# NVlabs/bayes-sim-ig

Measured on AMD Instinct MI355X. Metric: summary_vectors_per_sec_in_fit, higher is better.
Workload: dtype f32; 1 GPU; cfg5: ShadowHand MDRFF-4096 K=4 D=32, summary_start (I=2310), 100000 pairs/GPU, reference chunk protocol: <=1000-pair chunks, summarizer + 100 Adam updates x minibatch 100 + 6 held-out evals per chunk; pairs_per_gpu=100000, parallelism=dp1, gradient_exchange=none, hip_graph=True

## Files before the change

bayes_sim_ig_amd/csrc/fit_deferred_eval.hip:

```cpp
#include "persist.h"

#include <algorithm>
#include <cstdlib>

#include "persist_linear_device.h"

namespace bsig {

struct DArgs {
  int e0, n_ev_chunk;
  float* slabs; int64_t slab_stride;
  float* rows; int row_floats;
  float* sx; float* sl;
};

__device__ __forceinline__ UEval d_eval_of(const UArgs& p, const DArgs& d, int gidx) {
  const int c = p.chunks ? gidx / d.n_ev_chunk : 0;
  return u_eval_of(p, c, gidx - c * d.n_ev_chunk);
}
__device__ __forceinline__ bool d_gave_up(const UArgs& p) {
  return (__hip_atomic_load(p.state + ST_FLAGS, __ATOMIC_RELAXED, __HIP_MEMORY_SCOPE_AGENT) & kFlagTimeout) != 0;
}
__device__ __forceinline__ float d_slot_sum(const float* vals, int n, int lane) {
  float v[4];
#pragma unroll
  for (int u = 0; u < 4; ++u) v[u] = lane + 64 * u < n ? vals[lane + 64 * u] : 0.f;
  return granule_slot_sum(v);
}

template <int NT>
__global__ __launch_bounds__(kUT) void deferred_eval_products_kernel(UArgs p, DArgs d) {
  extern __shared__ __attribute__((aligned(16))) float smem[];
#ifndef BSIG_HOST_SAN_BUILD
  if (d_gave_up(p)) return;
  constexpr int NBW = 16 * NT;
  float* Wl = smem;
  float* biasl = Wl + NBW * p.WP;
  const int tid = threadIdx.x;
  const int slot = blockIdx.x, gidx = d.e0 + blockIdx.y;
  const int ks = slot / p.n_blocks, nb = slot - ks * p.n_blocks;
  const float* src = p.snap + ((int64_t)gidx * p.G + slot) * u_snap_slot_floats(NT, p.WP);
  const int quads = NBW * p.WP / 4 + (ks == 0 ? NBW / 4 : 0);
  for (int i = tid; i < quads; i += kUT)
    *reinterpret_cast<f32x4*>(Wl + 4 * i) = *reinterpret_cast<const f32x4*>(src + 4 * i);
  __syncthreads();
  u_eval_products<NT>(p, Wl, biasl, ks, nb * NBW, ks * p.KS, d_eval_of(p, d, gidx), d.slabs + blockIdx.y * d.slab_stride);
#endif
}

__global__ __launch_bounds__(kUT) void deferred_eval_rows_kernel(UArgs p, DArgs d) {
  extern __shared__ __attribute__((aligned(16))) float smem[];
#ifndef BSIG_HOST_SAN_BUILD
  if (d_gave_up(p)) return;
  float* XS = smem;
  float* red = XS + d.row_floats;
  const int tid = threadIdx.x;
  const int eo = blockIdx.x, y = blockIdx.y;
  for (int i = tid; i < d.row_floats; i += kUT) XS[i] = 0.f;
  __syncthreads();
  const float sx = u_eval_rows(p, d.slabs + y * d.slab_stride, XS, red, eo, d_eval_of(p, d, d.e0 + y), tid);
  if (tid == 0) d.sx[y * p.NE + eo] = sx;
  float* out = d.rows + ((int64_t)y * p.NE + eo) * d.row_floats;
  for (int i = tid; i < d.row_floats; i += kUT) out[i] = XS[i];
#endif
}

__global__ __launch_bounds__(kUT) void deferred_eval_nll_kernel(UArgs p, DArgs d) {
  extern __shared__ __attribute__((aligned(16))) float smem[];
#ifndef BSIG_HOST_SAN_BUILD
  if (d_gave_up(p)) return;
  float* XS = smem;
  float* red = XS + d.row_floats;
  const int tid = threadIdx.x, lane = tid & 63;
  const int eo = blockIdx.x, y = blockIdx.y;
  const float* in = d.rows + ((int64_t)y * p.NE + eo) * d.row_floats;
  for (int i = tid; i < d.row_floats; i += kUT) XS[i] = in[i];
  __syncthreads();
  bool bad;
  const float sl = u_eval_nll(p, XS, red, eo, d_eval_of(p, d, d.e0 + y), u_head_args(p), tid,
                              [&] { return d_slot_sum(d.sx + y * p.NE, p.NE, lane); }, bad);
  if (tid == 0) d.sl[y * p.NE + eo] = sl;
  if (bad) atomicOr(p.state + ST_FLAGS, kFlagNonfinite);
#endif
}

__global__ __launch_bounds__(64) void deferred_eval_log_kernel(UArgs p, DArgs d, int n) {
#ifndef BSIG_HOST_SAN_BUILD
  if (d_gave_up(p)) return;
  const int lane = threadIdx.x;
  for (int y = 0; y < n; ++y) {
    const float sum = d_slot_sum(d.sl + y * p.NE, p.NE, lane);
    if (lane == 0) u_eval_log(p, d_eval_of(p, d, d.e0 + y), sum, p.state + ST_FLAGS);
  }
#endif
}

namespace {
struct DLayout { size_t snap_off, snap_bytes, slab_off, rows_off, sx_off, sl_off, total; int group; size_t slab_stride; int row_floats; };

DLayout d_layout(const UGeom& g, int n_evals) {
  DLayout L{};
  L.snap_off = 256;
  L.snap_bytes = round_up<size_t>(deferred_eval_snapshot_bytes(g, n_evals), 256);
  L.slab_stride = (size_t)std::max(g.eval_passes, 1) * g.slab_floats;
  L.group = (int)std::max<size_t>(1, std::min<size_t>({(size_t)n_evals, (size_t)64,
                                                      kDeferredGroupBytes / std::max<size_t>(L.slab_stride * sizeof(float), 1)}));
  L.row_floats = (int)round_up(g.RE * g.per_wave, 4);
  L.slab_off = L.snap_off + L.snap_bytes;
  L.rows_off = L.slab_off + round_up<size_t>((size_t)L.group * L.slab_stride * sizeof(float), 256);
  L.sx_off = L.rows_off + round_up<size_t>((size_t)L.group * g.NE * L.row_floats * sizeof(float), 256);
  L.sl_off = L.sx_off + round_up<size_t>((size_t)L.group * g.NE * sizeof(float), 256);
  L.total = L.sl_off + round_up<size_t>((size_t)L.group * g.NE * sizeof(float), 256);
  return L;
}
}

size_t deferred_eval_snapshot_bytes(const UGeom& g, int n_evals) {
  return (size_t)n_evals * g.G * (size_t)u_snap_slot_floats(g.NT, g.WP) * sizeof(float);
}

bool deferred_eval_reserve(const UGeom& g, int n_evals, DeferredEval* d) {
  if (n_evals < 1 || g.eval_passes < 1) return false;
  size_t cap = kDeferredSnapCapBytes;
  if (const char* e = getenv("BSIG_DEFERRED_EVAL_CAP_MB")) cap = (size_t)std::max(atoll(e), 0ll) << 20;
  if (deferred_eval_snapshot_bytes(g, n_evals) > cap) return false;
  if (d->mem && d->n_evals >= n_evals) return true;
  const DLayout L = d_layout(g, n_evals);
  if (d->mem) {
    if (hipDeviceSynchronize() != hipSuccess || hipFree(d->mem) != hipSuccess) return false;
    *d = DeferredEval{};
  }
  void* mem = nullptr;
  if (hipMalloc(&mem, L.total) != hipSuccess) {
    (void)hipGetLastError();
    return false;
  }
  d->mem = mem; d->bytes = L.total; d->n_evals = n_evals;
  return true;
}

void deferred_eval_free(DeferredEval* d) {
  if (d->mem) (void)hipFree(d->mem);
  *d = DeferredEval{};
}

int deferred_eval_run(const PersistShape& s, const UGeom& g, const PersistBuffers& b, int n, hipStream_t st) {
  BSIG_REQUIRE(b.deferred && b.do_eval && n >= 1, "deferred evaluations: not a launch with snapshots");
  UArgs p;
  BSIG_TRY(persist_fill_args(s, g, b, n, &p));
  const int n_ev_chunk = (int)count_logging_points(n);
  const int n_evals = n_ev_chunk * (b.chunks ? b.n_chunks : 1);
  const DLayout L = d_layout(g, n_evals);
  char* base = reinterpret_cast<char*>(b.deferred);
  DArgs d{};
  d.n_ev_chunk = n_ev_chunk;
  d.slabs = reinterpret_cast<float*>(base + L.slab_off); d.slab_stride = (int64_t)L.slab_stride;
  d.rows = reinterpret_cast<float*>(base + L.rows_off); d.row_floats = L.row_floats;
  d.sx = reinterpret_cast<float*>(base + L.sx_off); d.sl = reinterpret_cast<float*>(base + L.sl_off);
  const size_t lds_tile = (size_t)u_snap_slot_floats(g.NT, g.WP) * sizeof(float);
  const size_t lds_rows = ((size_t)L.row_floats + 64) * sizeof(float);
  BSIG_REQUIRE(lds_tile <= kLdsUnraised && lds_rows <= kLdsUnraised, "deferred evaluations: tile or rows beyond 64 KB of LDS");
  for (int e0 = 0; e0 < n_evals; e0 += L.group) {
    const int ne = std::min(L.group, n_evals - e0);
    d.e0 = e0;
    if (g.NT == 1)
      hipLaunchKernelGGL((deferred_eval_products_kernel<1>), dim3(g.G, ne), dim3(kUT), lds_tile, st, p, d);
    else
      hipLaunchKernelGGL((deferred_eval_products_kernel<2>), dim3(g.G, ne), dim3(kUT), lds_tile, st, p, d);
    BSIG_CHECK_LAUNCH("deferred_eval_products");
    hipLaunchKernelGGL(deferred_eval_rows_kernel, dim3(g.NE, ne), dim3(kUT), lds_rows, st, p, d);
    BSIG_CHECK_LAUNCH("deferred_eval_rows");
    hipLaunchKernelGGL(deferred_eval_nll_kernel, dim3(g.NE, ne), dim3(kUT), lds_rows, st, p, d);
    BSIG_CHECK_LAUNCH("deferred_eval_nll");
    hipLaunchKernelGGL(deferred_eval_log_kernel, dim3(1), dim3(64), 0, st, p, d, ne);
    BSIG_CHECK_LAUNCH("deferred_eval_log");
  }
  return BSIG_OK;
}

}
```

bayes_sim_ig_amd/csrc/persist.h:

```cpp
#pragma once
#include "common.h"

namespace bsig {

struct PersistEngine {
  int kind = 0;
  bool streams = false;
  bool eval_single = false;
  bool eval_dp = false;
  bool block_launch = false;
  size_t workspace_bytes = 0;
};

inline bool block_launch_resolved(int kind, bool eval_single, bool forced_single) {
  return kind == 1 && eval_single && !forced_single;
}

struct PersistShape {
  int batch, feat_dim, out_dim, n_comp;
  int max_test = 0;
};

struct UGeom {
  int NT, Bp, MT, FP, KS, ksteps, KB, WP, Nh, NhP, n_blocks, k_slices, G, T, n_owner, R;
  int per_wave, xs_floats;
  int eval_passes, NE, RE;
  size_t lds, slab_floats, dout_floats, eval_floats;
};

struct PersistHyper {
  double lr, beta1, beta2; float adam_eps, eps_noise, min_weight, ll_limit;
  int64_t norm_batch;
};

struct PersistCommon {
  const float* y; int64_t ldy;
  const int32_t* ids;
  float* params; float* exp_avg; float* exp_avg_sq;
  int32_t* state;
  float* train_loss;
  void* workspace; size_t workspace_bytes;
  float* grads = nullptr; int adam_pending = 0;
  unsigned* xr_ready = nullptr; const unsigned* xr_done = nullptr; unsigned xr_base = 0;
  int do_eval = 0; int eval_every = 1; int n_total = 0; int n_test = 0;
  const float* y_test = nullptr; int64_t ldy_test = 0;
  float* test_loss = nullptr;
  PersistHyper hy;
};

struct PersistBuffers : PersistCommon {
  const float* feats; int64_t ld_feats;
  const int32_t* feat_ids;
  int64_t w_off, b_off;
  int64_t eval_row0 = 0;
  const bsig_fit_chunk* chunks = nullptr; int n_chunks = 1;
  void* deferred = nullptr;
};

struct DeferredEval { void* mem = nullptr; size_t bytes = 0; int n_evals = 0; };
constexpr size_t kDeferredSnapCapBytes = (size_t)2 << 30;
constexpr size_t kDeferredGroupBytes = (size_t)96 << 20;
size_t deferred_eval_snapshot_bytes(const UGeom& g, int n_evals);
bool deferred_eval_reserve(const UGeom& g, int n_evals, DeferredEval* d);
void deferred_eval_free(DeferredEval* d);
int deferred_eval_run(const PersistShape& s, const UGeom& g, const PersistBuffers& b, int n, hipStream_t st);

bool persist_resolve(const PersistShape& s, UGeom* g, PersistEngine* e);
struct ZeroRegion { void* ptr; size_t bytes; };
int persist_reset_regions(const UGeom& g, void* workspace, size_t workspace_bytes, ZeroRegion* regions);
int persist_run(const PersistShape& s, const UGeom& g, const PersistBuffers& b, int n, hipStream_t st);

int persist_geometry(const PersistShape& s, int32_t* out);

template <int N>
inline int allow_dynamic_lds(LdsRaised (&raised)[N], const void* const (&kernels)[N], int bytes) {
  for (int i = 0; i < N; ++i) BSIG_TRY(raise_lds_limit(kernels[i], bytes, &raised[i]));
  return BSIG_OK;
}

void persist_set_profile_buffer(void* buf);
int debug_spin(int blocks, size_t lds_bytes, int ms, hipStream_t st);
void* persist_profile_buffer();

}
```

bayes_sim_ig_amd/csrc/persist_linear_device.h:

```cpp
#pragma once
#include "persist.h"
#include "head_device.h"
#include "persist_device.h"

namespace bsig {

constexpr int kUT = 512;
constexpr int kUSteps = 18;
constexpr int kUGroup = 6;
constexpr int kUMT = 7;
constexpr int kUProf = 8;
constexpr int kUFP = 116;

struct UArgs {
  int B, Bp, MT;
  int Fdim, KS, ksteps, KB, WP;
  int Nh, NhP, D, K;
  int n_blocks, k_slices, G, T, n_owner, R;
  int n_updates, xs_floats;
  int fast_rows;
  const float* feats; int64_t ld_feats; const int32_t* feat_ids;
  const float* y; int64_t ldy; const int32_t* ids;
  float* params; float* m1; float* m2; int64_t w_off, b_off;
  int32_t* state; float* train_loss;
  double lr, beta1, beta2;
  float adam_eps, eps_noise, min_w, ll_limit, inv_norm;
  float* slabs; float* d_out; float* e_out; unsigned* flag_fwd; unsigned long long* gran;
  unsigned long long* gran_rep;
  float* grads; int adam_pending; int quad_ok;
  unsigned* xr_ready; const unsigned* xr_done; unsigned* xr_count; unsigned xr_base;
  int do_eval, eval_every, n_total, n_test, eval_passes, NE, RE;
  int64_t eval_row0;
  const float* y_test; int64_t ldy_test;
  float* test_loss;
  float* eval_slabs;
  unsigned* flag_eval;
  unsigned long long* gran_eval;
  long long* prof;
  int prof_t0;
  const bsig_fit_chunk* chunks; int n_chunks;
  float* snap;
  const int32_t* state_in;
};
int persist_fill_args(const PersistShape& s, const UGeom& g, const PersistBuffers& b, int n, UArgs* out);
__host__ __device__ inline int64_t u_snap_slot_floats(int NT, int WP) { return (int64_t)16 * NT * (WP + 1); }

struct UCk {
  int step0, n_updates, n_total, eval_every, do_eval;
  unsigned ubase, evbase;
  uint64_t seed, rng_ctr0;
};
__device__ __forceinline__ int u_uniform(int v) { return __builtin_amdgcn_readfirstlane(v); }
__device__ __forceinline__ int64_t u_uniform(int64_t v) {
  return (int64_t)(((uint64_t)(uint32_t)u_uniform((int)((uint64_t)v >> 32)) << 32) | (uint32_t)u_uniform((int)(uint64_t)v));
}
__device__ __forceinline__ void u_chunk_load(const UArgs& p, int c, UCk& k) {
  if (p.chunks == nullptr) {
    k.step0 = p.state[ST_STEP]; k.n_updates = p.n_updates; k.n_total = p.n_total; k.eval_every = p.eval_every;
    k.do_eval = p.do_eval; k.ubase = 0u; k.evbase = 0u;
    k.seed = st_rng(p.state)[0];
    k.rng_ctr0 = st_rng(p.state)[1];
    return;
  }
  const bsig_fit_chunk& e = p.chunks[c];
  k.step0 = 0; k.n_updates = u_uniform(e.n_updates); k.n_total = k.n_updates; k.eval_every = u_uniform(e.eval_every);
  k.do_eval = 1; k.ubase = (unsigned)u_uniform(e.upd_base); k.evbase = (unsigned)u_uniform(e.eval_base);
  k.seed = (uint64_t)u_uniform((int64_t)e.seed); k.rng_ctr0 = (uint64_t)u_uniform((int64_t)e.rng_ctr0);
}

struct UEval {
  int n_test, passes; int64_t row0;
  const float* y_test; int64_t ldy_test;
  float* out;
  unsigned gidx;
  uint64_t seed, stream;
};
__device__ __forceinline__ UEval u_eval_of(const UArgs& p, int c, int e) {
  UEval v;
  int every, n_total, step0;
  uint64_t ctr0;
  if (p.chunks == nullptr) {
    v.n_test = p.n_test; v.row0 = p.eval_row0; v.y_test = p.y_test; v.ldy_test = p.ldy_test; v.out = nullptr;
    v.gidx = (unsigned)e; every = p.eval_every; n_total = p.n_total; step0 = p.state_in[ST_STEP];
    v.seed = st_rng(p.state_in)[0];
    ctr0 = st_rng(p.state_in)[1];
  } else {
    const bsig_fit_chunk& k = p.chunks[c];
    v.n_test = u_uniform(k.n_test); v.row0 = u_uniform(k.row0) + u_uniform(k.n_train);
    v.y_test = p.y + v.row0 * p.ldy; v.ldy_test = p.ldy; v.out = p.test_loss + u_uniform(k.test_slot) + e;
    v.gidx = (unsigned)u_uniform(k.eval_base) + (unsigned)e; every = u_uniform(k.eval_every);
    n_total = u_uniform(k.n_updates); step0 = 0;
    v.seed = (uint64_t)u_uniform((int64_t)k.seed); ctr0 = (uint64_t)u_uniform((int64_t)k.rng_ctr0);
  }
  v.passes = (v.n_test + p.B - 1) / p.B;
  const int at = eval_at_step(e, every, n_total);
  const int ev0 = p.do_eval || p.chunks ? evals_before(step0, every) : 0;
  v.stream = launch_stream(ctr0, at - step0, e, ev0);
  return v;
}

__device__ __forceinline__ f32x4 umfma(float a, float b, f32x4 c) {
  return __builtin_amdgcn_mfma_f32_16x16x4f32(a, b, c, 0, 0, 0);
}

template <typename RowOff, typename F>
__device__ __forceinline__ void u_rows_sum(const float* slabs, RowOff&& rowoff, int k_slices, int zs, int nrows,
                                           int n_cols, float* out, int out_pitch, int tid, F&& fn) {
  const __amdgpu_buffer_rsrc_t sr = xwg_buffer(slabs);
  for (int idx = tid; idx < nrows * n_cols; idx += kUT) {
    const int r = idx / n_cols, col = idx - r * n_cols;
    const int voff = (rowoff(r) + col) * 4;
    float v = 0.f;
    for (int z = 0; z < k_slices; z += 16) {
      float q[16];
#pragma unroll
      for (int u = 0; u < 16; ++u)
        q[u] = __uint_as_float(__builtin_amdgcn_raw_buffer_load_b32(sr, voff, min(z + u, k_slices - 1) * zs * 4, kXwgPolicy));
#pragma unroll
      for (int u = 0; u < 16; ++u)
        if (z + u < k_slices) v += q[u];
    }
    out[r * out_pitch + col] = v;
    fn(col, v);
  }
}


template <int NT>
__device__ __forceinline__ void u_eval_products(const UArgs& p, const float* Wl, const float* biasl, int ks, int n0,
                                                int k0, const UEval& ev, float* ebase) {
  int tid = threadIdx.x;
  asm volatile("" : "+v"(tid));
  const int lane = tid & 63, w = tid >> 6, c16 = lane & 15, g4 = lane >> 4;
  const int B = p.B, NhP = p.NhP;
  for (int pass = 0; pass < ev.passes; ++pass) {
    const int rows = min(B, ev.n_test - pass * B);
    if (rows <= 0) break;
    if (w < p.MT) {
      f32x4 acc[NT];
#pragma unroll
      for (int nt = 0; nt < NT; ++nt) {
        const f32x4 zero = {0.f, 0.f, 0.f, 0.f};
        acc[nt] = ks == 0 ? *reinterpret_cast<const f32x4*>(biasl + 16 * nt + 4 * g4) : zero;
      }
      const int64_t r = ev.row0 + pass * B + min(16 * w + c16, rows - 1);
      const float* src = p.feats + r * p.ld_feats;
      const float* ap = Wl + c16 * p.WP + 4 * g4;
#pragma unroll 1
      for (int s0 = 0; s0 < p.ksteps; s0 += kUGroup) {
        f32x4 breg[kUGroup];
#pragma unroll
        for (int q = 0; q < kUGroup; ++q) {
          const int col = k0 + 16 * (s0 + q) + 4 * g4;
          const f32x4 v = *reinterpret_cast<const f32x4*>(src + min((int64_t)col, p.ld_feats - 4));
          const f32x4 zero = {0.f, 0.f, 0.f, 0.f};
          breg[q] = col < p.Fdim ? v : zero;
        }
#pragma unroll
        for (int q = 0; q < kUGroup; ++q) {
#pragma unroll
          for (int nt = 0; nt < NT; ++nt) {
            const f32x4 a4 = *reinterpret_cast<const f32x4*>(ap + nt * 16 * p.WP + 16 * (s0 + q));
            acc[nt] = umfma(a4[0], breg[q][0], acc[nt]);
            acc[nt] = umfma(a4[1], breg[q][1], acc[nt]);
            acc[nt] = umfma(a4[2], breg[q][2], acc[nt]);
            acc[nt] = umfma(a4[3], breg[q][3], acc[nt]);
          }
        }
      }
      if (16 * w + c16 < rows) {
        const __amdgpu_buffer_rsrc_t sr = xwg_buffer(ebase + (((int64_t)pass * p.k_slices + ks) * B) * NhP + n0);
#pragma unroll
        for (int nt = 0; nt < NT; ++nt)
          xwg_store4(sr, (16 * w + c16) * NhP + 16 * nt + 4 * g4, acc[nt][0], acc[nt][1], acc[nt][2], acc[nt][3]);
      }
    }
  }
}

__device__ __forceinline__ float u_eval_rows(const UArgs& p, const float* ebase, float* XS, float* red, int eo,
                                             const UEval& ev, int tid) {
  const int lane = tid & 63, w = tid >> 6;
  const int B = p.B, Nh = p.Nh, NhP = p.NhP, K = p.K, DK = p.D * p.K;
  const int per_wave = Nh + p.D + 3 * K;
  const int nr = eo < ev.n_test ? min(p.RE, (ev.n_test - eo + p.NE - 1) / p.NE) : 0;
  float eacc = 0.f;
  u_rows_sum(ebase,
             [&](int r) {
               const int erow = eo + p.NE * r, pass = erow / B, rb = erow - pass * B;
               return (pass * p.k_slices * B + rb) * NhP;
             },
             p.k_slices, B * NhP, nr, Nh, XS, per_wave, tid,
             [&](int col, float v) { if (col >= K + DK && col < K + 2 * DK) eacc += expf(v); });
  eacc = wave_sum_dpp(eacc);
  if (lane == 0) red[w] = eacc;
  __syncthreads();
  float sx = 0.f;
  if (tid == 0)
    for (int q = 0; q < kUT / 64; ++q) sx += red[q];
  return sx;
}

template <typename SumExp>
__device__ __forceinline__ float u_eval_nll(const UArgs& p, float* XS, float* red, int eo, const UEval& ev,
                                            const HeadArgs& a, int tid, SumExp&& sum_exp, bool& bad) {
  const int lane = tid & 63, w = tid >> 6;
  const int Nh = p.Nh, D = p.D, K = p.K, DK = D * K;
  const int per_wave = Nh + D + 3 * K;
  const int nr = eo < ev.n_test ? min(p.RE, (ev.n_test - eo + p.NE - 1) / p.NE) : 0;
  const int erow = eo + p.NE * w;
  const bool act = w < nr;
  float* tile = XS + w * per_wave;
  float* yv = tile + Nh;
  float* rk = yv + D;
  float* lpk = rk + K;
  float* dlg = lpk + K;
  if (act)
    for (int j = lane; j < D; j += 64) yv[j] = ev.y_test[(int64_t)erow * ev.ldy_test + j];
  RowOut ro;
  ro.lse = 0.f; ro.uds = 0.f; ro.bad = false;
#pragma unroll
  for (int q = 0; q < kElemsPerLane; ++q) ro.esg0[q] = 0.f;
  if (w < p.RE) {
    HeadArgs ae = a;
    ae.d_out = nullptr;
    ae.batch = ev.n_test;
    ae.seed = ev.seed;
    ae.stream_id = ev.stream;
    diag_row(ae, erow, act, lane, tile, yv, rk, lpk, dlg,
             [&] {
               return p.eps_noise != 0.f ? p.eps_noise * (sum_exp() / ((float)ev.n_test * (float)DK)) : 0.f;
             },
             ro);
  }
  if (lane == 0) red[16 + w] = act ? ro.lse : 0.f;
  __syncthreads();
  float sl = 0.f;
  if (tid == 0)
    for (int q = 0; q < kUT / 64; ++q) sl += red[16 + q];
  bad = ro.bad;
  return sl;
}

__device__ __forceinline__ void u_eval_log(const UArgs& p, const UEval& ev, float sum, int32_t* flagp) {
  const float l = -sum / (float)ev.n_test;
  if (ev.out) *ev.out = l;
  else p.test_loss[p.state[ST_EVAL]] = l;
  p.state[ST_EVAL] = p.state[ST_EVAL] + 1;
  if (!isfinite(l)) atomicOr(flagp, kFlagNonfinite);
}

__device__ __forceinline__ HeadArgs u_head_args(const UArgs& p) {
  HeadArgs a{};
  a.D = p.D; a.K = p.K; a.Nh = p.Nh; a.batch = p.B; a.from_tuple = 0;
  a.min_w = p.min_w; a.ll_limit = p.ll_limit; a.inv_norm = p.inv_norm;
  a.eps_noise = p.eps_noise; a.d_out = p.d_out;
  return a;
}

template <int NT>
__device__ __forceinline__ void u_tile_eval(const UArgs& p, const float* Wl, const float* biasl, int slot,
                                            int ks, int n0, int k0, const UEval& ev) {
  u_eval_products<NT>(p, Wl, biasl, ks, n0, k0, ev,
                      p.eval_slabs + (int64_t)(ev.gidx % 3u) * p.eval_passes * p.k_slices * p.B * p.NhP);
  __builtin_amdgcn_s_waitcnt(0);
  __syncthreads();
  if (threadIdx.x == 0) flag_raise(p.flag_eval, slot, ev.gidx + 1u);
}

__device__ __forceinline__ void u_owner_eval(const UArgs& p, float* XS, float* red, int eo, const UEval& ev,
                                             const HeadArgs& a) {
  int tid = threadIdx.x;
  asm volatile("" : "+v"(tid));
  const int lane = tid & 63, w = tid >> 6;
  int32_t* flagp = p.state + ST_FLAGS;
  const unsigned etag = ev.gidx + 1u;
  if (w == 0) flags_wait(p.flag_eval, p.G, etag, lane, flagp);
  __syncthreads();
  const float* ebase = p.eval_slabs + (int64_t)(ev.gidx % 3u) * p.eval_passes * p.k_slices * p.B * p.NhP;
  const float sx = u_eval_rows(p, ebase, XS, red, eo, ev, tid);
  if (tid == 0) granule_publish(p.gran_eval, eo, etag, sx);
  bool bad;
  const float sl = u_eval_nll(p, XS, red, eo, ev, a, tid,
                              [&] { return granule_gather(p.gran_eval, p.NE, etag, lane, flagp); }, bad);
  if (tid == 0) granule_publish(p.gran_eval + kGranArr, eo, etag, sl);
  if (eo == 0 && w == 0) {
    const float sum = granule_gather(p.gran_eval + kGranArr, p.NE, etag, lane, flagp);
    if (lane == 0) u_eval_log(p, ev, sum, flagp);
  }
  if (bad) atomicOr(flagp, kFlagNonfinite);
  __syncthreads();
}

}
```

Measured before the change: 584,400 pairs/s.

## Restructure deferred eval products to reduce k-slices in-block with double-buffered tiles

The deferred-evaluation products kernel now launches one block per (eval, row group, n-block). Each block loops over all k-slices, streaming the weight tiles through double-buffered LDS with register prefetch and software-pipelined feature loads. It accumulates the k-slice partial sums in registers and writes one reduced sums buffer, instead of per-k-slice slabs that the rows kernel previously summed. The smaller intermediate lets group sizes grow (up to 4096 evals), which cuts launches, and the log kernel is parallelized across evals when chunked. The cost is less grid parallelism over k-slices and more register pressure.

New measurement: 588,200 pairs/s (median of 2 runs). About the same (+0.6%).

```diff
diff --git a/bayes_sim_ig_amd/csrc/fit_deferred_eval.hip b/bayes_sim_ig_amd/csrc/fit_deferred_eval.hip
--- a/bayes_sim_ig_amd/csrc/fit_deferred_eval.hip
+++ b/bayes_sim_ig_amd/csrc/fit_deferred_eval.hip
@@ -7,9 +7,14 @@
 
 namespace bsig {
 
+constexpr int kDRounds = 2;
+constexpr int kDRows = 16 * kDRounds * (kUT / 64);
+constexpr int kDQuads = 4;
+
 struct DArgs {
-  int e0, n_ev_chunk;
-  float* slabs; int64_t slab_stride;
+  int e0, n, n_ev_chunk;
+  int n_rg, lds_bufs;
+  float* sums; int64_t sum_stride;
   float* rows; int row_floats;
   float* sx; float* sl;
 };
@@ -34,17 +39,97 @@
 #ifndef BSIG_HOST_SAN_BUILD
   if (d_gave_up(p)) return;
   constexpr int NBW = 16 * NT;
-  float* Wl = smem;
-  float* biasl = Wl + NBW * p.WP;
-  const int tid = threadIdx.x;
-  const int slot = blockIdx.x, gidx = d.e0 + blockIdx.y;
-  const int ks = slot / p.n_blocks, nb = slot - ks * p.n_blocks;
-  const float* src = p.snap + ((int64_t)gidx * p.G + slot) * u_snap_slot_floats(NT, p.WP);
-  const int quads = NBW * p.WP / 4 + (ks == 0 ? NBW / 4 : 0);
-  for (int i = tid; i < quads; i += kUT)
-    *reinterpret_cast<f32x4*>(Wl + 4 * i) = *reinterpret_cast<const f32x4*>(src + 4 * i);
+  const int tid = threadIdx.x, lane = tid & 63, w = u_uniform(tid >> 6), c16 = lane & 15, g4 = lane >> 4;
+  const int item = blockIdx.x;
+  const int y = item / (d.n_rg * p.n_blocks), rg = (item - y * d.n_rg * p.n_blocks) / p.n_blocks;
+  const int nb = item - (y * d.n_rg + rg) * p.n_blocks;
+  const int gidx = d.e0 + y;
+  const UEval ev = d_eval_of(p, d, gidx);
+  const int rows = min(kDRows, ev.n_test - rg * kDRows);
+  if (rows <= 0) return;
+  const int n_mt = (rows + 15) / 16;
+  const int mt[kDRounds] = {w, kUT / 64 + w};
+  const bool has[kDRounds] = {mt[0] < n_mt, mt[1] < n_mt};
+  const int64_t slot_floats = u_snap_slot_floats(NT, p.WP);
+  const float* tiles = p.snap + ((int64_t)gidx * p.G + nb) * slot_floats;
+  const int64_t tile_step = (int64_t)p.n_blocks * slot_floats;
+  const float* biasl = smem + NBW * p.WP;
+  f32x4 pre[kDQuads];
+  auto tile_request = [&](int ks) {
+    const int quads = NBW * p.WP / 4 + (ks == 0 ? NBW / 4 : 0);
+    const float* src = tiles + ks * tile_step;
+#pragma unroll
+    for (int u = 0; u < kDQuads; ++u) {
+      const int i = tid + u * kUT;
+      if (i < quads) pre[u] = *reinterpret_cast<const f32x4*>(src + 4 * i);
+    }
+  };
+  auto tile_to_lds = [&](int ks) {
+    const int quads = NBW * p.WP / 4 + (ks == 0 ? NBW / 4 : 0);
+    float* dst = smem + (ks & (d.lds_bufs - 1)) * slot_floats;
+#pragma unroll
+    for (int u = 0; u < kDQuads; ++u) {
+      const int i = tid + u * kUT;
+      if (i < quads) *reinterpret_cast<f32x4*>(dst + 4 * i) = pre[u];
+    }
+  };
+  tile_request(0);
+  const int64_t row0 = ev.row0 + rg * kDRows;
+  const float* frow[kDRounds];
+#pragma unroll
+  for (int r = 0; r < kDRounds; ++r) frow[r] = u_slice_row(p, row0, rows, 16 * mt[r] + c16);
+  f32x4 cur[kUGroup];
+  u_slice_operands(p, frow[0], 0, 0, g4, cur);
+  tile_to_lds(0);
   __syncthreads();
-  u_eval_products<NT>(p, Wl, biasl, ks, nb * NBW, ks * p.KS, d_eval_of(p, d, gidx), d.slabs + blockIdx.y * d.slab_stride);
+  f32x4 sum[kDRounds][NT];
+#pragma unroll
+  for (int r = 0; r < kDRounds; ++r)
+#pragma unroll
+    for (int nt = 0; nt < NT; ++nt) sum[r][nt] = f32x4{0.f, 0.f, 0.f, 0.f};
+#pragma unroll 1
+  for (int ks = 0; ks < p.k_slices; ++ks) {
+    const bool more = ks + 1 < p.k_slices;
+    const int k0 = ks * p.KS;
+    if (more) tile_request(ks + 1);
+    const float* ap = smem + (ks & (d.lds_bufs - 1)) * slot_floats + c16 * p.WP + 4 * g4;
+#pragma unroll
+    for (int r = 0; r < kDRounds; ++r) {
+      if (!has[r]) continue;
+      f32x4 acc[NT];
+      u_slice_start<NT>(biasl, ks, g4, acc);
+#pragma unroll 1
+      for (int s0 = 0; s0 < p.ksteps; s0 += kUGroup) {
+        const bool same = s0 + kUGroup < p.ksteps, other = !same && r + 1 < kDRounds && has[r + 1 < kDRounds ? r + 1 : r];
+        const float* nrow = same ? frow[r] : other ? frow[r + 1 < kDRounds ? r + 1 : r] : frow[0];
+        const int nk0 = same || other || !more ? k0 : k0 + p.KS;
+        f32x4 nxt[kUGroup];
+        u_slice_request(p, nrow, nk0, same ? s0 + kUGroup : 0, g4, nxt);
+        __builtin_amdgcn_sched_barrier(0);
+        u_slice_mfmas<NT>(p, ap, s0, cur, acc);
+        __builtin_amdgcn_sched_barrier(0);
+        u_slice_arrived(p, nk0, same ? s0 + kUGroup : 0, g4, nxt);
+#pragma unroll
+        for (int q = 0; q < kUGroup; ++q) cur[q] = nxt[q];
+      }
+#pragma unroll
+      for (int nt = 0; nt < NT; ++nt)
+#pragma unroll
+        for (int i = 0; i < 4; ++i) sum[r][nt][i] += acc[nt][i];
+    }
+    if (d.lds_bufs == 1) __syncthreads();
+    if (more) tile_to_lds(ks + 1);
+    __syncthreads();
+  }
+  float* out = d.sums + y * d.sum_stride + (int64_t)rg * kDRows * p.NhP + nb * NBW;
+#pragma unroll
+  for (int r = 0; r < kDRounds; ++r) {
+    const int mrow = 16 * mt[r] + c16;
+    if (has[r] && mrow < rows) {
+#pragma unroll
+      for (int nt = 0; nt < NT; ++nt) *reinterpret_cast<f32x4*>(out + (int64_t)mrow * p.NhP + 16 * nt + 4 * g4) = sum[r][nt];
+    }
+  }
 #endif
 }
 
@@ -58,7 +143,9 @@
   const int eo = blockIdx.x, y = blockIdx.y;
   for (int i = tid; i < d.row_floats; i += kUT) XS[i] = 0.f;
   __syncthreads();
-  const float sx = u_eval_rows(p, d.slabs + y * d.slab_stride, XS, red, eo, d_eval_of(p, d, d.e0 + y), tid);
+  UArgs q = p;
+  q.k_slices = 1;
+  const float sx = u_eval_rows(q, d.sums + y * d.sum_stride, XS, red, eo, d_eval_of(p, d, d.e0 + y), tid);
   if (tid == 0) d.sx[y * p.NE + eo] = sx;
   float* out = d.rows + ((int64_t)y * p.NE + eo) * d.row_floats;
   for (int i = tid; i < d.row_floats; i += kUT) out[i] = XS[i];
@@ -84,11 +171,17 @@
 #endif
 }
 
-__global__ __launch_bounds__(64) void deferred_eval_log_kernel(UArgs p, DArgs d, int n) {
+__global__ __launch_bounds__(64) void deferred_eval_log_kernel(UArgs p, DArgs d) {
 #ifndef BSIG_HOST_SAN_BUILD
   if (d_gave_up(p)) return;
   const int lane = threadIdx.x;
-  for (int y = 0; y < n; ++y) {
+  if (p.chunks) {
+    const int y = blockIdx.x;
+    const float sum = d_slot_sum(d.sl + y * p.NE, p.NE, lane);
+    if (lane == 0) u_eval_log(p, d_eval_of(p, d, d.e0 + y), sum, p.state + ST_FLAGS, y == 0 ? d.n : 0);
+    return;
+  }
+  for (int y = 0; y < d.n; ++y) {
     const float sum = d_slot_sum(d.sl + y * p.NE, p.NE, lane);
     if (lane == 0) u_eval_log(p, d_eval_of(p, d, d.e0 + y), sum, p.state + ST_FLAGS);
   }
@@ -96,18 +189,18 @@
 }
 
 namespace {
-struct DLayout { size_t snap_off, snap_bytes, slab_off, rows_off, sx_off, sl_off, total; int group; size_t slab_stride; int row_floats; };
+struct DLayout { size_t snap_off, snap_bytes, sums_off, rows_off, sx_off, sl_off, total; int group; size_t sum_stride; int row_floats; };
 
 DLayout d_layout(const UGeom& g, int n_evals) {
   DLayout L{};
   L.snap_off = 256;
   L.snap_bytes = round_up<size_t>(deferred_eval_snapshot_bytes(g, n_evals), 256);
-  L.slab_stride = (size_t)std::max(g.eval_passes, 1) * g.slab_floats;
-  L.group = (int)std::max<size_t>(1, std::min<size_t>({(size_t)n_evals, (size_t)64,
-                                                      kDeferredGroupBytes / std::max<size_t>(L.slab_stride * sizeof(float), 1)}));
+  L.sum_stride = (size_t)std::max(g.eval_passes, 1) * g.dout_floats;
   L.row_floats = (int)round_up(g.RE * g.per_wave, 4);
-  L.slab_off = L.snap_off + L.snap_bytes;
-  L.rows_off = L.slab_off + round_up<size_t>((size_t)L.group * L.slab_stride * sizeof(float), 256);
+  const size_t per_eval = (L.sum_stride + (size_t)g.NE * L.row_floats + 2 * (size_t)g.NE) * sizeof(float);
+  L.group = (int)std::max<size_t>(1, std::min<size_t>({(size_t)n_evals, (size_t)kDeferredGroupMax, kDeferredRowsBytes / per_eval}));
+  L.sums_off = L.snap_off + L.snap_bytes;
+  L.rows_off = L.sums_off + round_up<size_t>((size_t)L.group * L.sum_stride * sizeof(float), 256);
   L.sx_off = L.rows_off + round_up<size_t>((size_t)L.group * g.NE * L.row_floats * sizeof(float), 256);
   L.sl_off = L.sx_off + round_up<size_t>((size_t)L.group * g.NE * sizeof(float), 256);
   L.total = L.sl_off + round_up<size_t>((size_t)L.group * g.NE * sizeof(float), 256);
@@ -154,25 +247,30 @@
   char* base = reinterpret_cast<char*>(b.deferred);
   DArgs d{};
   d.n_ev_chunk = n_ev_chunk;
-  d.slabs = reinterpret_cast<float*>(base + L.slab_off); d.slab_stride = (int64_t)L.slab_stride;
+  d.n_rg = ceil_div(b.n_test, kDRows);
+  d.sums = reinterpret_cast<float*>(base + L.sums_off); d.sum_stride = (int64_t)L.sum_stride;
   d.rows = reinterpret_cast<float*>(base + L.rows_off); d.row_floats = L.row_floats;
   d.sx = reinterpret_cast<float*>(base + L.sx_off); d.sl = reinterpret_cast<float*>(base + L.sl_off);
   const size_t lds_tile = (size_t)u_snap_slot_floats(g.NT, g.WP) * sizeof(float);
   const size_t lds_rows = ((size_t)L.row_floats + 64) * sizeof(float);
   BSIG_REQUIRE(lds_tile <= kLdsUnraised && lds_rows <= kLdsUnraised, "deferred evaluations: tile or rows beyond 64 KB of LDS");
+  BSIG_REQUIRE(lds_tile <= (size_t)kDQuads * kUT * 16 && b.n_test <= g.eval_passes * s.batch,
+               "deferred evaluations: tile beyond a workgroup's copy, or more held-out rows than the plan's");
+  d.lds_bufs = 2 * lds_tile <= kLdsUnraised ? 2 : 1;
   for (int e0 = 0; e0 < n_evals; e0 += L.group) {
     const int ne = std::min(L.group, n_evals - e0);
-    d.e0 = e0;
+    d.e0 = e0; d.n = ne;
+    const int blocks = ne * d.n_rg * g.n_blocks;
     if (g.NT == 1)
-      hipLaunchKernelGGL((deferred_eval_products_kernel<1>), dim3(g.G, ne), dim3(kUT), lds_tile, st, p, d);
+      hipLaunchKernelGGL((deferred_eval_products_kernel<1>), dim3(blocks), dim3(kUT), d.lds_bufs * lds_tile, st, p, d);
     else
-      hipLaunchKernelGGL((deferred_eval_products_kernel<2>), dim3(g.G, ne), dim3(kUT), lds_tile, st, p, d);
+      hipLaunchKernelGGL((deferred_eval_products_kernel<2>), dim3(blocks), dim3(kUT), d.lds_bufs * lds_tile, st, p, d);
     BSIG_CHECK_LAUNCH("deferred_eval_products");
     hipLaunchKernelGGL(deferred_eval_rows_kernel, dim3(g.NE, ne), dim3(kUT), lds_rows, st, p, d);
     BSIG_CHECK_LAUNCH("deferred_eval_rows");
     hipLaunchKernelGGL(deferred_eval_nll_kernel, dim3(g.NE, ne), dim3(kUT), lds_rows, st, p, d);
     BSIG_CHECK_LAUNCH("deferred_eval_nll");
-    hipLaunchKernelGGL(deferred_eval_log_kernel, dim3(1), dim3(64), 0, st, p, d, ne);
+    hipLaunchKernelGGL(deferred_eval_log_kernel, dim3(b.chunks ? ne : 1), dim3(64), 0, st, p, d);
     BSIG_CHECK_LAUNCH("deferred_eval_log");
   }
   return BSIG_OK;
diff --git a/bayes_sim_ig_amd/csrc/persist.h b/bayes_sim_ig_amd/csrc/persist.h
--- a/bayes_sim_ig_amd/csrc/persist.h
+++ b/bayes_sim_ig_amd/csrc/persist.h
@@ -59,7 +59,8 @@
 
 struct DeferredEval { void* mem = nullptr; size_t bytes = 0; int n_evals = 0; };
 constexpr size_t kDeferredSnapCapBytes = (size_t)2 << 30;
-constexpr size_t kDeferredGroupBytes = (size_t)96 << 20;
+constexpr size_t kDeferredRowsBytes = (size_t)96 << 20;
+constexpr int kDeferredGroupMax = 4096;
 size_t deferred_eval_snapshot_bytes(const UGeom& g, int n_evals);
 bool deferred_eval_reserve(const UGeom& g, int n_evals, DeferredEval* d);
 void deferred_eval_free(DeferredEval* d);
diff --git a/bayes_sim_ig_amd/csrc/persist_linear_device.h b/bayes_sim_ig_amd/csrc/persist_linear_device.h
--- a/bayes_sim_ig_amd/csrc/persist_linear_device.h
+++ b/bayes_sim_ig_amd/csrc/persist_linear_device.h
@@ -127,6 +127,68 @@
 
 
 template <int NT>
+__device__ __forceinline__ void u_slice_start(const float* biasl, int ks, int g4, f32x4 (&acc)[NT]) {
+#pragma unroll
+  for (int nt = 0; nt < NT; ++nt) {
+    const f32x4 zero = {0.f, 0.f, 0.f, 0.f};
+    acc[nt] = ks == 0 ? *reinterpret_cast<const f32x4*>(biasl + 16 * nt + 4 * g4) : zero;
+  }
+}
+__device__ __forceinline__ void u_slice_request(const UArgs& p, const float* src, int k0, int s0, int g4,
+                                                f32x4 (&breg)[kUGroup]) {
+#pragma unroll
+  for (int q = 0; q < kUGroup; ++q) {
+    const int col = k0 + 16 * (s0 + q) + 4 * g4;
+    breg[q] = *reinterpret_cast<const f32x4*>(src + min((int64_t)col, p.ld_feats - 4));
+  }
+}
+__device__ __forceinline__ void u_slice_arrived(const UArgs& p, int k0, int s0, int g4, f32x4 (&breg)[kUGroup]) {
+#pragma unroll
+  for (int q = 0; q < kUGroup; ++q) {
+    const int col = k0 + 16 * (s0 + q) + 4 * g4;
+    const f32x4 zero = {0.f, 0.f, 0.f, 0.f};
+    breg[q] = col < p.Fdim ? breg[q] : zero;
+  }
+}
+__device__ __forceinline__ void u_slice_operands(const UArgs& p, const float* src, int k0, int s0, int g4,
+                                                 f32x4 (&breg)[kUGroup]) {
+  u_slice_request(p, src, k0, s0, g4, breg);
+  u_slice_arrived(p, k0, s0, g4, breg);
+}
+template <int NT>
+__device__ __forceinline__ void u_slice_mfmas(const UArgs& p, const float* ap, int s0, const f32x4 (&breg)[kUGroup],
+                                              f32x4 (&acc)[NT]) {
+#pragma unroll
+  for (int q = 0; q < kUGroup; ++q) {
+#pragma unroll
+    for (int nt = 0; nt < NT; ++nt) {
+      const f32x4 a4 = *reinterpret_cast<const f32x4*>(ap + nt * 16 * p.WP + 16 * (s0 + q));
+      acc[nt] = umfma(a4[0], breg[q][0], acc[nt]);
+      acc[nt] = umfma(a4[1], breg[q][1], acc[nt]);
+      acc[nt] = umfma(a4[2], breg[q][2], acc[nt]);
+      acc[nt] = umfma(a4[3], breg[q][3], acc[nt]);
+    }
+  }
+}
+__device__ __forceinline__ const float* u_slice_row(const UArgs& p, int64_t row0, int rows, int mrow) {
+  return p.feats + (row0 + min(mrow, rows - 1)) * p.ld_feats;
+}
+template <int NT>
+__device__ __forceinline__ void u_slice_products(const UArgs& p, const float* Wl, const float* biasl, int ks, int k0,
+                                                 int64_t row0, int rows, int mrow0, int lane, f32x4 (&acc)[NT]) {
+  const int c16 = lane & 15, g4 = lane >> 4;
+  u_slice_start<NT>(biasl, ks, g4, acc);
+  const float* src = u_slice_row(p, row0, rows, mrow0 + c16);
+  const float* ap = Wl + c16 * p.WP + 4 * g4;
+#pragma unroll 1
+  for (int s0 = 0; s0 < p.ksteps; s0 += kUGroup) {
+    f32x4 breg[kUGroup];
+    u_slice_operands(p, src, k0, s0, g4, breg);
+    u_slice_mfmas<NT>(p, ap, s0, breg, acc);
+  }
+}
+
+template <int NT>
 __device__ __forceinline__ void u_eval_products(const UArgs& p, const float* Wl, const float* biasl, int ks, int n0,
                                                 int k0, const UEval& ev, float* ebase) {
   int tid = threadIdx.x;
@@ -138,36 +200,7 @@
     if (rows <= 0) break;
     if (w < p.MT) {
       f32x4 acc[NT];
-#pragma unroll
-      for (int nt = 0; nt < NT; ++nt) {
-        const f32x4 zero = {0.f, 0.f, 0.f, 0.f};
-        acc[nt] = ks == 0 ? *reinterpret_cast<const f32x4*>(biasl + 16 * nt + 4 * g4) : zero;
-      }
-      const int64_t r = ev.row0 + pass * B + min(16 * w + c16, rows - 1);
-      const float* src = p.feats + r * p.ld_feats;
-      const float* ap = Wl + c16 * p.WP + 4 * g4;
-#pragma unroll 1
-      for (int s0 = 0; s0 < p.ksteps; s0 += kUGroup) {
-        f32x4 breg[kUGroup];
-#pragma unroll
-        for (int q = 0; q < kUGroup; ++q) {
-          const int col = k0 + 16 * (s0 + q) + 4 * g4;
-          const f32x4 v = *reinterpret_cast<const f32x4*>(src + min((int64_t)col, p.ld_feats - 4));
-          const f32x4 zero = {0.f, 0.f, 0.f, 0.f};
-          breg[q] = col < p.Fdim ? v : zero;
-        }
-#pragma unroll
-        for (int q = 0; q < kUGroup; ++q) {
-#pragma unroll
-          for (int nt = 0; nt < NT; ++nt) {
-            const f32x4 a4 = *reinterpret_cast<const f32x4*>(ap + nt * 16 * p.WP + 16 * (s0 + q));
-            acc[nt] = umfma(a4[0], breg[q][0], acc[nt]);
-            acc[nt] = umfma(a4[1], breg[q][1], acc[nt]);
-            acc[nt] = umfma(a4[2], breg[q][2], acc[nt]);
-            acc[nt] = umfma(a4[3], breg[q][3], acc[nt]);
-          }
-        }
-      }
+      u_slice_products<NT>(p, Wl, biasl, ks, k0, ev.row0 + pass * B, rows, 16 * w, lane, acc);
       if (16 * w + c16 < rows) {
         const __amdgpu_buffer_rsrc_t sr = xwg_buffer(ebase + (((int64_t)pass * p.k_slices + ks) * B) * NhP + n0);
 #pragma unroll
@@ -242,11 +275,11 @@
   return sl;
 }
 
-__device__ __forceinline__ void u_eval_log(const UArgs& p, const UEval& ev, float sum, int32_t* flagp) {
+__device__ __forceinline__ void u_eval_log(const UArgs& p, const UEval& ev, float sum, int32_t* flagp, int advance = 1) {
   const float l = -sum / (float)ev.n_test;
   if (ev.out) *ev.out = l;
   else p.test_loss[p.state[ST_EVAL]] = l;
-  p.state[ST_EVAL] = p.state[ST_EVAL] + 1;
+  if (advance) p.state[ST_EVAL] = p.state[ST_EVAL] + advance;
   if (!isfinite(l)) atomicOr(flagp, kFlagNonfinite);
 }
 
```
